# mynameisfiber/baton

Hardware: NVIDIA H100
Metric: federated local samples/sec (whole box), ResNet-18 FedAvg, synthetic non-IID 32x32 shards (higher is better)
Workload: dtype bf16

## Files before the change

### baton_b200/csrc/bindings.cpp

```cpp
#include <ATen/cuda/CUDAContext.h>
#include <c10/cuda/CUDAGuard.h>
#include <torch/extension.h>

#include <optional>
#include <vector>

#include "launch.h"

namespace {

inline cudaStream_t cur_stream() { return at::cuda::getCurrentCUDAStream().stream(); }
inline void check(int rc, const char* what) {
  TORCH_CHECK(rc == 0, "baton_b200::", what, " failed with code ", rc,
              rc > 0 ? std::string(" (") + cudaGetErrorString(static_cast<cudaError_t>(rc)) + ")" : std::string());
}
inline const void* cptr(const at::Tensor& t) { return t.data_ptr(); }
inline void* ptr(at::Tensor& t) { return t.data_ptr(); }
template <class T>
inline T* opt_ptr(const std::optional<at::Tensor>& t) {
  return (t.has_value() && t->defined()) ? reinterpret_cast<T*>(t->data_ptr()) : nullptr;
}
#define CHECK_CUDA(x) TORCH_CHECK((x).is_cuda(), #x " must be a CUDA tensor")

inline const float* prox_anchor(const std::optional<at::Tensor>& anchor, int64_t numel, const at::Tensor& hyper) {
// ... 239 lines not shown
                                static_cast<int>(stride), dgrad ? 1 : 0, static_cast<int>(mc), opt_ptr<float>(col_stats),
                                cur_stream());
  if (rc == -2) return false;
  check(rc, "conv_halo");
  return true;
}
bool conv_igemm_dgrad_s2(const at::Tensor& dy, const at::Tensor& w, at::Tensor dx, int64_t kh, int64_t kw,
                         const std::vector<int64_t>& ntaps, const std::vector<int64_t>& taps, int64_t force_bn) {
  CHECK_CUDA(dy); CHECK_CUDA(w); CHECK_CUDA(dx);
  TORCH_CHECK(dy.scalar_type() == at::kBFloat16 && w.scalar_type() == at::kBFloat16 && dx.scalar_type() == at::kBFloat16 &&
              dy.dim() == 4 && dx.dim() == 4 && dy.is_contiguous() && w.is_contiguous() && dx.is_contiguous());
  TORCH_CHECK(ntaps.size() == 4 && taps.size() == 16, "conv_igemm_dgrad_s2: 4 classes x 4 taps");
  int nt[4], tw[16];
  for (int i = 0; i < 4; ++i) nt[i] = static_cast<int>(ntaps[i]);
  for (int i = 0; i < 16; ++i) tw[i] = static_cast<int>(taps[i]);
  const c10::cuda::CUDAGuard guard(dy.device());
  const int rc = b200_conv_igemm_dgrad_s2(cptr(dy), cptr(w), ptr(dx), static_cast<int>(dx.size(0)),
                                          static_cast<int>(dx.size(1)), static_cast<int>(dx.size(2)),
                                          static_cast<int>(dx.size(3)), static_cast<int>(dy.size(3)), static_cast<int>(kh),
                                          static_cast<int>(kw), static_cast<int>(dy.size(1)), static_cast<int>(dy.size(2)),
                                          nt, tw, static_cast<int>(force_bn), cur_stream());
  if (rc == -2) return false;
  check(rc, "conv_igemm_dgrad_s2");
  return true;
}
bool conv_igemm_wgrad(const at::Tensor& dy, const at::Tensor& x, at::Tensor dw, int64_t cout, int64_t kh, int64_t kw,
                      int64_t stride, int64_t pad, int64_t ho, int64_t wo, int64_t split_k, int64_t force_bn,
                      const std::optional<at::Tensor>& sgd_theta, const std::optional<at::Tensor>& sgd_theta_bf16,
                      const std::optional<at::Tensor>& sgd_mom, const std::optional<at::Tensor>& sgd_hyper,
                      bool sgd_nesterov, const std::optional<at::Tensor>& sgd_anchor,
                      const std::optional<at::Tensor>& sgd_corr, const std::optional<at::Tensor>& sgd_v) {
  CHECK_CUDA(dy); CHECK_CUDA(x); CHECK_CUDA(dw);
  TORCH_CHECK(x.scalar_type() == at::kBFloat16 && dy.scalar_type() == at::kBFloat16 && dw.scalar_type() == at::kFloat &&
              x.dim() == 4 && x.is_contiguous() && dy.is_contiguous());
  const c10::cuda::CUDAGuard guard(x.device());
  const std::optional<B200SgdEpilogue> sgd =
      sgd_epilogue(sgd_theta, sgd_theta_bf16, sgd_mom, sgd_hyper, sgd_nesterov, sgd_anchor, sgd_corr, sgd_v);
  const int rc = b200_conv_igemm_wgrad(cptr(dy), cptr(x), dw.data_ptr<float>(), static_cast<int>(x.size(0)),
                                       static_cast<int>(x.size(1)), static_cast<int>(x.size(2)), static_cast<int>(x.size(3)),
                                       static_cast<int>(cout), static_cast<int>(kh), static_cast<int>(kw),
                                       static_cast<int>(stride), static_cast<int>(pad), static_cast<int>(ho),
                                       static_cast<int>(wo), static_cast<int>(split_k), static_cast<int>(force_bn),
                                       sgd ? &*sgd : nullptr, cur_stream());
  if (rc == -2 || rc == B200_SGD_EPILOGUE_DECLINED) return false;
  check(rc, "conv_igemm_wgrad");
  return true;
// ... 886 lines not shown
  const c10::cuda::CUDAGuard guard(pred.device());
  const int in32 = pred.scalar_type() == at::kFloat;
  const int out32 = dpred.has_value() && dpred->defined() && dpred->scalar_type() == at::kFloat;
  check(b200_mse(pred.data_ptr(), in32, target.data_ptr<float>(), opt_ptr<void>(dpred), out32,
                 loss_acc.data_ptr<float>(), pred.numel(), static_cast<float>(grad_scale), cur_stream()),
        "mse");
}

}

PYBIND11_MODULE(TORCH_EXTENSION_NAME, m) {
  m.doc() = "baton_b200 sm_90a kernels";
  m.attr("MAX_RANKS") = B200_MAX_RANKS;
  m.def("gemm", &gemm);
  m.def("trace_set", &trace_set);
  m.def("attention_fwd", &attention_fwd);
  m.def("attention_bwd", &attention_bwd);
  m.def("bn_bwd_cluster", &bn_bwd_cluster);
  m.def("im2col_tma_probe", &im2col_tma_probe);
  m.def("conv_igemm_fwd", &conv_igemm_fwd);
  m.def("conv_igemm_wgrad", &conv_igemm_wgrad);
  m.def("conv_igemm_dgrad", &conv_igemm_dgrad);
  m.def("conv_igemm_dgrad_s2", &conv_igemm_dgrad_s2);
  m.def("conv_halo", &conv_halo);
  m.def("gemm_batched", &gemm_batched);
  m.def("gemm_fp8", &gemm_fp8);
  m.def("quant_mx_rows", &quant_mx_rows);
  m.def("quant_mx_cols", &quant_mx_cols);
  m.def("fused_sgd", &fused_sgd);
  m.def("fused_sgd_segments", &fused_sgd_segments);
  m.def("weighted_sum", &weighted_sum);
  m.def("fold_client", &fold_client);
  m.def("scaffold_corr", &scaffold_corr);
  m.def("scaffold_dc", &scaffold_dc);
  m.def("cast", &cast);
  m.def("gather_rows", &gather_rows);
  m.def("gather_augment", &gather_augment);
  m.def("gather_mix", &gather_mix);
  m.def("colsum", &colsum);
  m.def("add_bf16", &add_bf16);
  m.def("relu_bwd", &relu_bwd);
  m.def("gelu", &gelu);
  m.def("gelu_bwd", &gelu_bwd);
  m.def("pad_rows", &pad_rows);
  m.def("embedding_bwd", &embedding_bwd);
  m.def("fedavg_allreduce", &fedavg_allreduce);
// ... 41 lines not shown
```

### baton_b200/csrc/gemm_wgmma.cu

```cuda
#define B200_TU_TAG 1
#include "ptx.cuh"
#include "epilogue.cuh"
#include "launch.h"
#include "pdl.cuh"
#include "sgd.cuh"

namespace b200 {

constexpr int BM = 128;
constexpr int BK = 64;
constexpr int WG_K = 16;
constexpr int GEMM_THREADS = 384;
constexpr int CONSUMER_WARPS = 8;
constexpr int CONSUMER_THREADS = 32 * CONSUMER_WARPS;
constexpr int MAX_STAGES = 8;
constexpr int S2_MAX_TAPS = 4;

struct GemmParams {
  int M, N, K;
  void* D;
  long long ldd;
  const float* bias;
  int out_fp32;
  int act;
  float* col_stats;
  int a_mn, b_mn;
  int k_tiles_per_split;
  int atomic_out;
  int cluster_k;
  int stages;
  const uint32_t* tile_flags;
  uint32_t flag_epoch;
  long long flag_elem_off;
  int flag_tile_elems;
  long long flag_bias_off;
  long long ldb;
  float alpha;
  int batched, batch_inner;
  int batch_count;
  long long d_outer, d_inner;
  int conv_ho, conv_wo;
  int conv_stride, conv_pad;
  int conv_kw;
  int conv_cin;
  int conv_taps;
  int conv_ncol;
  const uint32_t* flag_epoch_ptr;
  const float* sgd_hyper = nullptr;
  float* sgd_theta = nullptr;
  __nv_bfloat16* sgd_wb = nullptr;
  float* sgd_mom = nullptr;
  int sgd_nesterov = 0;
  int conv_h = 0, conv_w = 0;
  int s2_ntaps[4] = {0, 0, 0, 0};
  int s2_tap[4][S2_MAX_TAPS] = {};
  const float* bn_scale = nullptr;
  const float* bn_shift = nullptr;
  const __nv_bfloat16* residual = nullptr;
  long long ldr = 0;
  const float* sgd_anchor = nullptr;
  const float* sgd_corr = nullptr;
  float* sgd_v = nullptr;
};

__device__ __forceinline__ void wait_arrival_flags(const uint32_t* flags, long long e0, long long e1, int granule,
                                                   uint32_t need) {
  for (long long t = e0 / granule; t <= e1 / granule; ++t) {
    unsigned long long spins = 0;
    while (static_cast<int32_t>(ld_acquire_sys(flags + t) - need) < 0) {
      if (++spins > (1ull << 26)) break;
    }
  }
}

template <int BN>
struct SmemLayout {
  static constexpr int A_BYTES = BM * BK * 2;
  static constexpr int B_BYTES = BN * BK * 2;
  static constexpr int STAGE_BYTES = A_BYTES + B_BYTES;
  static constexpr int PART_PITCH = BN + 4;
  static constexpr int PART_BYTES = BM * PART_PITCH * 4;
};

__device__ __forceinline__ float apply_act(float v, int act) {
  if (act == 1) return fmaxf(v, 0.f);
// ... 278 lines not shown
  return w;
}
__device__ __forceinline__ int s2_dx_row(const GemmParams& p, int cls, int m) {
  if (m >= p.M) return -1;
  const int hw = p.conv_ho * p.conv_wo;
  const int n = m / hw, r = m - n * hw;
  const int i = r / p.conv_wo, j = r - i * p.conv_wo;
  const int h = 2 * i + (cls >> 1), w = 2 * j + (cls & 1);
  return (h < p.conv_h && w < p.conv_w) ? (n * p.conv_h + h) * p.conv_w + w : -1;
}
template <int BN>
__device__ __forceinline__ void s2_load_ktile(const CUtensorMap* tmA, const CUtensorMap* tmB, const GemmParams& p,
                                              uint8_t* sa, uint8_t* sb, uint64_t* bar, int cls, int kt, int m0, int n0) {
  const int cblocks = p.conv_cin >> 6;
  const int slot = kt / cblocks, cb = kt - slot * cblocks;
  const int tw = s2_tap(p, cls, slot);
  const int q0 = m0 % p.conv_wo, t0 = m0 / p.conv_wo;
  tma_load_im2col_4d(sa, tmA, bar, cb * 64, q0, t0 % p.conv_ho, t0 / p.conv_ho, (tw >> 24) & 0xff, (tw >> 16) & 0xff);
  const int wcol = (tw & 0xffff) * p.conv_ncol + n0;
#pragma unroll
  for (int j = 0; j < BN / 64; ++j) tma_load_2d(sb + j * 8192, tmB, bar, wcol + j * 64, cb * 64);
}

template <int BN, int STAGES, int CONV = 0, bool SGD = false, bool AFFINE = false, bool PROX = false, bool SCAF = false,
          bool ADAM = false>
__global__ void __launch_bounds__(GEMM_THREADS, 1)
gemm_bf16_fixed_kernel(const __grid_constant__ CUtensorMap tmA, const __grid_constant__ CUtensorMap tmB,
                         const GemmParams p) {
  using L = SmemLayout<BN>;
  static_assert(STAGES * L::STAGE_BYTES >= L::PART_BYTES, "the drained ring must hold the fp32 accumulator tile");
  extern __shared__ __align__(1024) uint8_t smem_raw[];
  uint8_t* smem = reinterpret_cast<uint8_t*>((reinterpret_cast<uintptr_t>(smem_raw) + 1023) & ~uintptr_t(1023));
  uint64_t* full_bar = reinterpret_cast<uint64_t*>(smem + STAGES * L::STAGE_BYTES);
  uint64_t* empty_bar = full_bar + STAGES;
  float* cstat = reinterpret_cast<float*>(empty_bar + STAGES);

  griddep_launch_dependents();
  const int warp = threadIdx.x >> 5;
  int m0 = blockIdx.y * BM;
  const int cls = CONV == 4 ? s2_class(p, m0) : 0;
  const int n0 = blockIdx.x * BN;
  const int k_tiles_total = CONV == 4 ? s2_ntaps(p, cls) * (p.conv_cin >> 6) : (p.K + BK - 1) / BK;
  const int bz_outer = p.batched ? static_cast<int>(blockIdx.z) / p.batch_inner : 0;
  const int bz_inner = p.batched ? static_cast<int>(blockIdx.z) % p.batch_inner : 0;
  const int kt_begin = p.batched ? 0 : blockIdx.z * p.k_tiles_per_split;
  int kt_end = kt_begin + p.k_tiles_per_split;
  if (kt_end > k_tiles_total) kt_end = k_tiles_total;
  const int num_kt = kt_end - kt_begin;

  if (warp == 0 && elect_one()) {
    tma_prefetch_desc(&tmA);
    tma_prefetch_desc(&tmB);
    for (int s = 0; s < STAGES; ++s) {
      mbar_init(&full_bar[s], 1);
      mbar_init(&empty_bar[s], CONSUMER_WARPS);
    }
    fence_barrier_init();
  }
  __syncthreads();
  griddep_wait();

  if (warp == 0) {
    if (elect_one()) {
      if (p.tile_flags != nullptr) {
        const int rows_here = (p.N - n0) < BN ? (p.N - n0) : BN;
// ... 17 lines not shown
        if constexpr (CONV == 2) {
          const int live = (p.N - n0 + 63) / 64 < BN / 64 ? (p.N - n0 + 63) / 64 : BN / 64;
          mbar_expect_tx(&full_bar[s], L::A_BYTES + live * 8192);
        } else {
          mbar_expect_tx(&full_bar[s], L::STAGE_BYTES);
        }
        if (p.batched) {
          if (!p.a_mn) {
            tma_load_4d(sa, &tmA, &full_bar[s], k0, m0, bz_inner, bz_outer);
          } else {
#pragma unroll
            for (int j = 0; j < BM / 64; ++j)
              tma_load_4d(sa + j * 8192, &tmA, &full_bar[s], m0 + j * 64, k0, bz_inner, bz_outer);
          }
          if (!p.b_mn) {
            tma_load_4d(sb, &tmB, &full_bar[s], k0, n0, bz_inner, bz_outer);
          } else {
#pragma unroll
            for (int j = 0; j < BN / 64; ++j)
              tma_load_4d(sb + j * 8192, &tmB, &full_bar[s], n0 + j * 64, k0, bz_inner, bz_outer);
          }
        } else if constexpr (CONV == 4) {
          s2_load_ktile<BN>(&tmA, &tmB, p, sa, sb, &full_bar[s], cls, kt_begin + i, m0, n0);
        } else {
        if constexpr (CONV == 1 || CONV == 3) {
          const int kt = kt_begin + i;
          const int cblocks = p.conv_cin >> 6;
          const int tap = kt / cblocks, cb = kt - tap * cblocks;
          const int fr = tap / p.conv_kw, fs = tap - fr * p.conv_kw;
          const int q0 = m0 % p.conv_wo, t0 = m0 / p.conv_wo;
          tma_load_im2col_4d(sa, &tmA, &full_bar[s], cb * 64, q0 * p.conv_stride - p.conv_pad,
                             (t0 % p.conv_ho) * p.conv_stride - p.conv_pad, t0 / p.conv_ho, fs, fr);
        } else if (!p.a_mn) {
          tma_load_2d(sa, &tmA, &full_bar[s], k0, m0);
        } else {
#pragma unroll
          for (int j = 0; j < BM / 64; ++j)
            tma_load_2d(sa + j * 8192, &tmA, &full_bar[s], m0 + j * 64, k0);
        }
        if constexpr (CONV == 2) {
          const int q0 = k0 % p.conv_wo, t0 = k0 / p.conv_wo;
          const int w0 = q0 * p.conv_stride - p.conv_pad, h0 = (t0 % p.conv_ho) * p.conv_stride - p.conv_pad;
          const int img = t0 / p.conv_ho;
#pragma unroll
          for (int j = 0; j < BN / 64; ++j) {
            const int col = n0 + j * 64;
// ... 15 lines not shown
        } else {
#pragma unroll
          for (int j = 0; j < BN / 64; ++j) tma_load_2d(sb + j * 8192, &tmB, &full_bar[s], n0 + j * 64, k0);
        }
        }
      }
    }
  } else if (warp >= 4) {
    const int ew = warp - 4;
    float acc[BN / 2];
    int s = 0;
    uint32_t ph = 0;
    consume_ktiles<BN>(acc, smem, STAGES, full_bar, empty_bar, s, ph, num_kt, p.a_mn, p.b_mn, ew >> 2);
    if (threadIdx.x == 128) TRACE_POINT();
    named_bar_sync(1, CONSUMER_THREADS);
    float* part = reinterpret_cast<float*>(smem);
    wg_store_acc<BN>(acc, part, L::PART_PITCH, 64 * (ew >> 2));
    named_bar_sync(1, CONSUMER_THREADS);
    const int q = ew & 3;
    constexpr int NCHUNK = BN / 32;
    const int c_begin = (ew < 4 ? 0 : (NCHUNK + 1) / 2) * 32, c_end = (ew < 4 ? (NCHUNK + 1) / 2 : NCHUNK) * 32;
    const int lrow = q * 32 + static_cast<int>(lane_id());
    const int row = m0 + lrow;
    const int orow = CONV == 4 ? s2_dx_row(p, cls, row) : row;
    const bool row_ok = CONV == 4 ? orow >= 0 : row < p.M;
    const size_t elt = p.out_fp32 ? 4 : 2;
    uint8_t* drow = reinterpret_cast<uint8_t*>(p.D) +
                    (static_cast<size_t>(CONV == 4 && orow < 0 ? 0 : orow) * p.ldd + static_cast<size_t>(bz_outer) * p.d_outer +
                     static_cast<size_t>(bz_inner) * p.d_inner) * elt;
    const bool vec_ok = ((reinterpret_cast<uintptr_t>(p.D) & 15) == 0) && ((p.ldd * elt) % 16 == 0);
    const bool sgd_vec = SGD && (p.ldd % 4 == 0) &&
                         ((reinterpret_cast<uintptr_t>(p.sgd_theta) | reinterpret_cast<uintptr_t>(p.sgd_mom) |
                           (PROX ? reinterpret_cast<uintptr_t>(p.sgd_anchor) : 0) |
                           (SCAF ? reinterpret_cast<uintptr_t>(p.sgd_corr) : 0) |
                           (ADAM ? reinterpret_cast<uintptr_t>(p.sgd_v) : 0)) & 15) == 0 &&
                         (reinterpret_cast<uintptr_t>(p.sgd_wb) & 7) == 0;
    float* sstat = cstat + q * 2 * BN;
    const bool want_stats = p.col_stats != nullptr;
#pragma unroll 1
    for (int c = c_begin; c < c_end; c += 32) {
      uint32_t r[32];
      acc_ld_row32(part + lrow * L::PART_PITCH + c, r);
      const int col0 = n0 + c;
      float v[32];
#pragma unroll
      for (int j = 0; j < 32; ++j) v[j] = __uint_as_float(r[j]);
      if (col0 >= p.N) {
        if (want_stats) { sstat[c + lane_id()] = 0.f; sstat[BN + c + lane_id()] = 0.f; }
        continue;
      }
      if constexpr (AFFINE) {
// ... 230 lines not shown
      epilogue_tile<BN>(p, acc_tile, ew & 3, ew >> 2, m0, n0, epi_stage + ew * EPI_WARP_BYTES,
                        vec_ok && ((d_off * elt) & 15) == 0, d_off);
    }
  }
}


template <int BN, bool CLUSTER, int CONV = 0, bool AFFINE = false>
__global__ void __launch_bounds__(GEMM_THREADS, 1)
gemm_bf16_splitk_kernel(const __grid_constant__ CUtensorMap tmA, const __grid_constant__ CUtensorMap tmB,
                        const GemmParams p) {
  using L = SmemLayout<BN>;
  extern __shared__ __align__(1024) uint8_t smem_raw[];
  uint8_t* smem = reinterpret_cast<uint8_t*>((reinterpret_cast<uintptr_t>(smem_raw) + 1023) & ~uintptr_t(1023));
  const int STAGES = p.stages;
  const int ring_bytes = STAGES * L::STAGE_BYTES;
  const int data_bytes = L::PART_BYTES > ring_bytes ? L::PART_BYTES : ring_bytes;
  uint64_t* full_bar = reinterpret_cast<uint64_t*>(smem + data_bytes);
  uint64_t* empty_bar = full_bar + MAX_STAGES;
  float* cstat = reinterpret_cast<float*>(empty_bar + MAX_STAGES);

  griddep_launch_dependents();
  const int warp = threadIdx.x >> 5;
  const int m0 = blockIdx.y * BM;
  const int n0 = blockIdx.x * BN;
  const int k_tiles_total = (p.K + BK - 1) / BK;
  const int kt_begin = blockIdx.z * p.k_tiles_per_split;
  int kt_end = kt_begin + p.k_tiles_per_split;
  if (kt_end > k_tiles_total) kt_end = k_tiles_total;
  const int num_kt = kt_end - kt_begin;

  if (warp == 0 && elect_one()) {
    tma_prefetch_desc(&tmA);
    tma_prefetch_desc(&tmB);
    for (int s = 0; s < STAGES; ++s) {
      mbar_init(&full_bar[s], 1);
      mbar_init(&empty_bar[s], CONSUMER_WARPS);
    }
    fence_barrier_init();
  }
  __syncthreads();
  griddep_wait();

  if (warp == 0) {
    if (elect_one()) {
      if (p.tile_flags != nullptr) {
        const int rows_here = (p.N - n0) < BN ? (p.N - n0) : BN;
        const uint32_t need = p.flag_epoch_ptr != nullptr ? *reinterpret_cast<const volatile uint32_t*>(p.flag_epoch_ptr)
                                                          : p.flag_epoch;
        wait_arrival_flags(p.tile_flags, p.flag_elem_off + static_cast<long long>(n0) * p.ldb,
                           p.flag_elem_off + static_cast<long long>(n0 + rows_here) * p.ldb - 1, p.flag_tile_elems, need);
        if (p.flag_bias_off >= 0)
          wait_arrival_flags(p.tile_flags, p.flag_bias_off + n0, p.flag_bias_off + n0 + rows_here - 1,
                             p.flag_tile_elems, need);
        fence_proxy_async_all();
      }
      int s = 0;
      uint32_t ph = 0;
      for (int i = 0; i < num_kt; ++i) {
        mbar_wait(&empty_bar[s], ph ^ 1);
        uint8_t* sa = smem + s * L::STAGE_BYTES;
        uint8_t* sb = sa + L::A_BYTES;
        const int k0 = (kt_begin + i) * BK;
        mbar_expect_tx(&full_bar[s], L::STAGE_BYTES);
        if constexpr (CONV == 1 || CONV == 3) {
          const int kt = kt_begin + i;
          const int cblocks = p.conv_cin >> 6;
          const int tap = kt / cblocks, cb = kt - tap * cblocks;
          const int fr = tap / p.conv_kw, fs = tap - fr * p.conv_kw;
          const int q0 = m0 % p.conv_wo, t0 = m0 / p.conv_wo;
          tma_load_im2col_4d(sa, &tmA, &full_bar[s], cb * 64, q0 * p.conv_stride - p.conv_pad,
                             (t0 % p.conv_ho) * p.conv_stride - p.conv_pad, t0 / p.conv_ho, fs, fr);
        } else if (!p.a_mn) {
          tma_load_2d(sa, &tmA, &full_bar[s], k0, m0);
        } else {
#pragma unroll
          for (int j = 0; j < BM / 64; ++j)
            tma_load_2d(sa + j * 8192, &tmA, &full_bar[s], m0 + j * 64, k0);
        }
        if constexpr (CONV == 3) {
          const int kt = kt_begin + i;
          const int cblocks = p.conv_cin >> 6;
          const int tap = kt / cblocks, cb = kt - tap * cblocks;
          const int wcol = (p.conv_taps - 1 - tap) * p.conv_ncol + n0;
#pragma unroll
          for (int j = 0; j < BN / 64; ++j) tma_load_2d(sb + j * 8192, &tmB, &full_bar[s], wcol + j * 64, cb * 64);
        } else if (!p.b_mn) {
          tma_load_2d(sb, &tmB, &full_bar[s], k0, n0);
        } else {
#pragma unroll
          for (int j = 0; j < BN / 64; ++j) tma_load_2d(sb + j * 8192, &tmB, &full_bar[s], n0 + j * 64, k0);
        }
        if (++s == STAGES) { s = 0; ph ^= 1; }
      }
    }
  } else if (warp >= 4) {
    const int ew = warp - 4;
    float acc[BN / 2];
    int s = 0;
    uint32_t ph = 0;
    consume_ktiles<BN>(acc, smem, STAGES, full_bar, empty_bar, s, ph, num_kt, p.a_mn, p.b_mn, ew >> 2);
    named_bar_sync(1, CONSUMER_THREADS);
    float* part = reinterpret_cast<float*>(smem);
    wg_store_acc<BN>(acc, part, L::PART_PITCH, 64 * (ew >> 2));
    if constexpr (!CLUSTER) {
      named_bar_sync(1, CONSUMER_THREADS);
      const int q = ew & 3;
      constexpr int NCHUNK = BN / 32;
      const int c_begin = (ew < 4 ? 0 : (NCHUNK + 1) / 2) * 32, c_end = (ew < 4 ? (NCHUNK + 1) / 2 : NCHUNK) * 32;
      const int lrow = q * 32 + static_cast<int>(lane_id());
      const int row = m0 + lrow;
      const size_t elt = p.out_fp32 ? 4 : 2;
      const bool vec_ok = ((reinterpret_cast<uintptr_t>(p.D) & 15) == 0) && ((p.ldd * elt) % 16 == 0);
#pragma unroll 1
      for (int c = c_begin; c < c_end; c += 32) {
        const int col0 = n0 + c;
        if (row >= p.M || col0 >= p.N) continue;
        uint32_t r[32];
        acc_ld_row32(part + lrow * L::PART_PITCH + c, r);
        float v[32];
#pragma unroll
        for (int j = 0; j < 32; ++j) v[j] = __uint_as_float(r[j]);
        store_row_chunk<32, AFFINE>(p, row, col0, v, vec_ok);
      }
    }
  }

  if constexpr (CLUSTER) {
    const int S = p.cluster_k;
    cluster_sync_all();
    if (warp >= 4 && warp < 8) {
      const uint32_t me = cluster_ctarank();
      const int rows_per = BM / S;
      constexpr int CG = BN / 8;
      const int t = threadIdx.x - 128;
      const size_t elt = p.out_fp32 ? 4 : 2;
      const bool vec_ok = ((reinterpret_cast<uintptr_t>(p.D) & 15) == 0) && ((p.ldd * elt) % 16 == 0);
      const bool want_stats = p.col_stats != nullptr;
      float cs[8] = {0.f, 0.f, 0.f, 0.f, 0.f, 0.f, 0.f, 0.f}, cq[8] = {0.f, 0.f, 0.f, 0.f, 0.f, 0.f, 0.f, 0.f};
      for (int item = t; item < rows_per * CG; item += 128) {
        const int lrow = static_cast<int>(me) * rows_per + item / CG;
        const int c = (item % CG) * 8;
        const uint32_t laddr = smem_u32(smem) + static_cast<uint32_t>((lrow * L::PART_PITCH + c) * 4);
        float v[8] = {0.f, 0.f, 0.f, 0.f, 0.f, 0.f, 0.f, 0.f};
        for (int r = 0; r < S; ++r) {
          const float4 a = ld_dsmem_f4(laddr, r), b = ld_dsmem_f4(laddr + 16, r);
          v[0] += a.x; v[1] += a.y; v[2] += a.z; v[3] += a.w;
          v[4] += b.x; v[5] += b.y; v[6] += b.z; v[7] += b.w;
        }
        const int row = m0 + lrow, col0 = n0 + c;
        if (want_stats) {
#pragma unroll
          for (int j = 0; j < 8; ++j) {
            const float rnd = __bfloat162float(__float2bfloat16_rn(v[j]));
            cs[j] += rnd;
            cq[j] = fmaf(rnd, rnd, cq[j]);
          }
        }
        if (row < p.M && col0 < p.N) store_row_chunk<8, AFFINE>(p, row, col0, v, vec_ok);
      }
      if (want_stats) {
#pragma unroll
        for (int j = 0; j < 8; ++j) {
#pragma unroll
          for (int o = CG; o < 32; o <<= 1) {
            cs[j] += __shfl_xor_sync(0xffffffffu, cs[j], o);
            cq[j] += __shfl_xor_sync(0xffffffffu, cq[j], o);
          }
        }
        const int wq = t >> 5, ln = t & 31;
        if (ln < CG) {
#pragma unroll
          for (int j = 0; j < 8; ++j) {
            cstat[wq * 2 * BN + ln * 8 + j] = cs[j];
            cstat[wq * 2 * BN + BN + ln * 8 + j] = cq[j];
          }
        }
        named_bar_sync(2, 128);
        for (int i = t; i < 2 * BN; i += 128) {
          const int col = i < BN ? i : i - BN;
          if (n0 + col < p.N) {
            const float v = cstat[i] + cstat[2 * BN + i] + cstat[4 * BN + i] + cstat[6 * BN + i];
            atomicAdd(p.col_stats + (i < BN ? 0 : p.N) + n0 + col, v);
          }
        }
      }
    }
    cluster_sync_all();
  }
}


typedef CUresult (*EncodeTiledFn)(CUtensorMap*, CUtensorMapDataType, cuuint32_t, void*, const cuuint64_t*,
                                  const cuuint64_t*, const cuuint32_t*, const cuuint32_t*, CUtensorMapInterleave,
                                  CUtensorMapSwizzle, CUtensorMapL2promotion, CUtensorMapFloatOOBfill);

static EncodeTiledFn get_encode_fn() {
  static thread_local bool ctx_bound = false;
  if (!ctx_bound) {
    cudaFree(nullptr);
    ctx_bound = true;
  }
  static EncodeTiledFn fn = nullptr;
  if (fn == nullptr) {
    void* ptr = nullptr;
    cudaDriverEntryPointQueryResult qres;
    cudaError_t e = cudaGetDriverEntryPoint("cuTensorMapEncodeTiled", &ptr, cudaEnableDefault, &qres);
    if (e != cudaSuccess || qres != cudaDriverEntryPointSuccess || ptr == nullptr) return nullptr;
    fn = reinterpret_cast<EncodeTiledFn>(ptr);
  }
// ... 439 lines not shown
  }
  if (max_taps == 0) return -2;
  const int bn = clamp_bn(force_bn > 0 ? force_bn : (Cin > 64 ? 128 : 64));
  CUtensorMap ta, tb;
  int rc = b200_encode_map_im2col_bf16(&ta, dy, N, Ho, Wo, Cout, 1, 1, 1, 0, 64, BM);
  if (rc) return rc;
  rc = make_map(&tb, w, Cout, static_cast<long long>(KH) * KW * Cin, static_cast<long long>(KH) * KW * Cin, 64, BK);
  if (rc) return rc;
  const int k_tiles = max_taps * (Cout / 64);
  p.M = static_cast<int>(M); p.N = Cin; p.K = k_tiles * BK; p.D = dx; p.ldd = Cin; p.bias = nullptr; p.out_fp32 = 0;
  p.act = 0; p.a_mn = 0; p.b_mn = 1; p.k_tiles_per_split = k_tiles; p.cluster_k = 1; p.atomic_out = 0;
  p.col_stats = nullptr;
  p.tile_flags = nullptr; p.flag_epoch = 0; p.alpha = 1.0f; p.flag_elem_off = 0; p.flag_tile_elems = 0;
  p.ldb = static_cast<long long>(KH) * KW * Cin;
  p.flag_bias_off = -1; p.flag_epoch_ptr = nullptr;
  p.batched = 0; p.batch_inner = 1; p.batch_count = 1; p.d_outer = 0; p.d_inner = 0;
  p.conv_ho = Ho; p.conv_wo = Wo; p.conv_stride = 2; p.conv_pad = 0; p.conv_kw = KW; p.conv_cin = Cout;
  p.conv_taps = KH * KW; p.conv_ncol = Cin; p.conv_h = H; p.conv_w = W;
  dim3 grid((Cin + bn - 1) / bn, static_cast<unsigned>(4 * tiles_m), 1);
  if (bn == 128) return launch_fixed<128, 6, 4>(ta, tb, p, grid, stream);
  return launch_fixed<64, 8, 4>(ta, tb, p, grid, stream);
}

extern "C" int b200_conv_igemm_wgrad(const void* dy, const void* x, float* dw, int N, int H, int W, int Cin, int Cout,
                                     int KH, int KW, int stride, int pad, int Ho, int Wo, int split_k, int force_bn,
                                     const B200SgdEpilogue* sgd, cudaStream_t stream) {
  using namespace b200;
  const long long Mp = static_cast<long long>(N) * Ho * Wo;
  const int Kc = KH * KW * Cin;
  if (Mp <= 0 || Cout <= 0) return 0;
  if (Cin % 64 != 0 || Cout % 8 != 0 || Mp > (1ll << 30) || (reinterpret_cast<uintptr_t>(x) & 15) ||
      (reinterpret_cast<uintptr_t>(dy) & 15) || (reinterpret_cast<uintptr_t>(dw) & 15))
    return -2;
  const int bn = clamp_bn(force_bn > 0 ? force_bn : (Kc > 64 ? 128 : 64));
  CUtensorMap ta, tb;
  int rc = make_map(&ta, dy, Mp, Cout, Cout, 64, BK);
  if (rc) return rc;
  rc = b200_encode_map_im2col_bf16(&tb, x, N, H, W, Cin, KH, KW, stride, pad, 64, 64);
  if (rc) return rc;
  const int k_tiles = static_cast<int>((Mp + BK - 1) / BK);
  if (split_k < 1) split_k = 1;
  if (split_k > k_tiles) split_k = k_tiles;
  const int per = (k_tiles + split_k - 1) / split_k;
  split_k = (k_tiles + per - 1) / per;
  if (sgd != nullptr && split_k != 1) return B200_SGD_EPILOGUE_DECLINED;
  GemmParams p;
// ... 21 lines not shown
```

### baton_b200/csrc/launch.h

```cpp
#pragma once
#include <cuda_runtime.h>
#include <stdint.h>

#define B200_MAX_RANKS 16

extern "C" {

struct B200SgdEpilogue {
  float* theta;
  void* theta_bf16;
  float* mom;
  const float* hyper;
  int nesterov;
  const float* anchor;
  const float* corr;
  float* v;
};
#define B200_SGD_EPILOGUE_DECLINED (-6)

struct B200AffineEpilogue {
  const float* scale;
  const float* shift;
  const void* residual;
  long long ldr;
// ... 1 lines not shown
};
#define B200_AFFINE_EPILOGUE_DECLINED (-7)

int b200_gemm_bf16(const void* a, const void* b, void* d, const float* bias, int M, int N, int K, long long lda,
                   long long ldb, long long ldd, int a_mn, int b_mn, int out_fp32, int act, int split_k, int accumulate,
                   float alpha, const uint32_t* tile_flags, uint32_t flag_epoch, long long flag_elem_off, int flag_tile_elems,
                   long long flag_bias_off, int force_bn, float* col_stats, const uint32_t* flag_epoch_ptr,
                   const B200SgdEpilogue* sgd, const B200AffineEpilogue* affine, cudaStream_t stream);
int b200_gemm_bf16_batched(const void* a, const void* b, void* d, int M, int N, int K, long long lda, long long ldb,
                           long long ldd, int a_mn, int b_mn, int out_fp32, int act, float alpha, int n_outer,
                           int n_inner, long long a_outer, long long a_inner, long long b_outer, long long b_inner,
                           long long d_outer, long long d_inner, int accumulate, cudaStream_t stream);
int b200_attention_fwd(const void* qkv, void* out, void* probs, int B, int S, int H, int dh, float scale,
                       cudaStream_t stream);
int b200_attention_bwd(const void* qkv, const void* dout, const void* probs, void* dqkv, int B, int S, int H, int dh,
                       float scale, cudaStream_t stream);
int b200_conv_igemm_fwd(const void* x, const void* w, void* y, int N, int H, int W, int Cin, int Cout, int KH, int KW,
                        int stride, int pad, int Ho, int Wo, int cluster_k, int force_bn, float* col_stats,
                        const B200AffineEpilogue* affine, cudaStream_t stream);
int b200_conv_igemm_dgrad(const void* dy, const void* w, void* dx, int N, int H, int W, int Cin, int Cout, int KH, int KW,
                          int pad, int Ho, int Wo, int cluster_k, int force_bn, cudaStream_t stream);
int b200_conv_igemm_dgrad_s2(const void* dy, const void* w, void* dx, int N, int H, int W, int Cin, int Cout, int KH,
                             int KW, int Ho, int Wo, const int* ntaps, const int* taps, int force_bn, cudaStream_t stream);
int b200_conv_igemm_wgrad(const void* dy, const void* x, float* dw, int N, int H, int W, int Cin, int Cout, int KH, int KW,
                          int stride, int pad, int Ho, int Wo, int split_k, int force_bn, const B200SgdEpilogue* sgd,
                          cudaStream_t stream);
int b200_conv_halo(const void* src, const void* w, void* out, int N, int H, int W, int C, int Nout, int stride,
                   int dgrad, int mc, float* col_stats, cudaStream_t stream);
int b200_im2col_tma_probe(const void* x, void* col, int N, int H, int W, int C, int KH, int KW, int stride, int pad,
                          int Ho, int Wo, cudaStream_t stream);
int b200_gemm_fp8(const void* a, const void* b, void* d, const float* bias, const void* sfa, const void* sfb, int M, int N,
                  int K, long long lda, long long ldb, long long ldd, int out_fp32, int act, int split_k, int accumulate,
                  float alpha, cudaStream_t stream);
int b200_quant_mx_rows(const void* x, void* q, void* sf, long long R, int C, long long ld_in, int Cp, cudaStream_t stream);
int b200_quant_mx_cols(const void* x, void* q, void* sf, long long R, int C, long long ld_in, long long Rp,
                       cudaStream_t stream);
int b200_gemm_simt(const void* a, const void* b, void* d, const float* bias, int M, int N, int K, long long lda,
                   long long ldb, long long ldd, int a_mn, int b_mn, int out_fp32, int act, int accumulate,
                   float alpha, cudaStream_t stream);

int b200_fused_sgd(float* w, float* g, float* mom, void* w_bf16, long long n, const float* hyper, int zero_grad,
                   int nesterov, const unsigned long long* wire_slot, const float* pack_global,
                   const float* pack_scale, long long n_pack, int wire_fp32, const float* prox_anchor,
                   const float* corr, float* adam_v, cudaStream_t stream);
int b200_fused_sgd_segments(float* w, float* g, float* mom, void* w_bf16, const long long* segments, int n_seg,
                            const float* hyper, int nesterov, const float* prox_anchor, const float* corr,
// ... 192 lines not shown
```

### baton_b200/ops/functional.py

```python
from __future__ import annotations

import collections
import functools
from typing import List, Optional, Sequence, Tuple

import torch

from ._ext import load

BF16 = torch.bfloat16
NUM_SMS = 132


def _pitch(t: torch.Tensor) -> int:
    assert t.dim() == 2 and (t.stride(1) == 1 or t.shape[1] == 1), "GEMM operand must have unit inner stride"
    return t.stride(0) if t.shape[0] > 1 else max(t.stride(0), t.shape[1])


def _tma_ok(t: torch.Tensor) -> bool:
    return t.dtype == BF16 and _pitch(t) % 8 == 0 and t.data_ptr() % 16 == 0


def pick_bn(M: int, N: int) -> int:
    m_tiles = (M + 127) // 128
# ... 387 lines not shown


def halo_smem_bytes(h: int, w: int, c: int = 64, stride: int = 1) -> int:
    ho, wo = conv_out_size(h, 3, stride, 1), conv_out_size(w, 3, stride, 1)
    box = (HALO_BM // (ho * wo)) * (stride * (ho - 1) + 3) * (stride * (wo - 1) + 3) * 128
    k_tiles = 9 * (c // 64)
    return c // 64 * round_up(box, 1024) + k_tiles * 8192 + round_up(1 + k_tiles, 16) * 8 + 4 * 64 * 4 + 1024


def halo_eligible(kh: int, kw: int, stride: int, pad: int, c: int, h: int, w: int,
                  affine: Optional[dict] = None, dgrad: bool = False) -> bool:
    if kh != 3 or kw != 3 or pad != 1 or (stride, c) not in _HALO_FORMS or (dgrad and stride != 1):
        return False
    hw = conv_out_size(h, 3, stride, 1) * conv_out_size(w, 3, stride, 1)
    return (hw <= HALO_BM and HALO_BM % hw == 0 and affine is None and
            halo_smem_bytes(h, w, c, stride) <= _HALO_MAX_SMEM)


def halo_cluster(m_rows: int) -> int:
    tiles = (m_rows + HALO_BM - 1) // HALO_BM
    return 4 if tiles % 4 == 0 else 2 if tiles % 2 == 0 else 1


def _conv_path(path: Optional[str], eligible: bool) -> str:
    if path is None:
        return "halo" if eligible else "im2col"
    if path not in ("halo", "im2col"):
        raise ValueError("path must be None, 'halo' or 'im2col', not {!r}".format(path))
    if path == "halo" and not eligible:
        raise ValueError("the halo kernel does not take this convolution (see halo_eligible)")
    return path


def conv_igemm_fwd(x: torch.Tensor, w2d: torch.Tensor, kh: int, kw: int, stride: int, pad: int,
                   col_stats: Optional[torch.Tensor] = None, affine: Optional[dict] = None,
                   cluster_k: Optional[int] = None, force_bn: int = 0,
                   out: Optional[torch.Tensor] = None, path: Optional[str] = None,
                   mc: Optional[int] = None) -> Optional[torch.Tensor]:
    n, h, w, c = x.shape
    cout = w2d.shape[0]
    if c % 64 or w2d.shape[1] != kh * kw * c or not x.is_contiguous() or not w2d.is_contiguous():
        return None
    ho, wo = conv_out_size(h, kh, stride, pad), conv_out_size(w, kw, stride, pad)
    M, K = n * ho * wo, kh * kw * c
    halo = halo_eligible(kh, kw, stride, pad, c, h, w, affine) and cout % 8 == 0
    if _conv_path(path, halo) == "halo":
        y = out if out is not None else torch.empty((M, cout), dtype=BF16, device=x.device)
        if not load().conv_halo(x, w2d, y, stride, False, mc or halo_cluster(M), col_stats):
            raise RuntimeError("conv_halo declined a convolution halo_eligible admits")
        return y
    bn = force_bn or pick_bn(M, cout)
    if cluster_k is None:
        cluster_k = pick_cluster_k(M, cout, K, bn)
    y = out if out is not None else torch.empty((M, cout), dtype=BF16, device=x.device)
    af = affine or {}
    ok = load().conv_igemm_fwd(x, w2d, y, kh, kw, stride, pad, ho, wo, cluster_k, bn, col_stats, af.get("scale"),
                               af.get("shift"), af.get("residual"), bool(af.get("relu", False)))
    return y if ok else None


S2_MAX_TAPS = 4


def conv_s2_dgrad_taps(kh: int, kw: int, pad: int, ho: int, wo: int) -> Optional[List[List[Tuple[int, int, int]]]]:
    classes = []
    for a in (0, 1):
        for b in (0, 1):
            taps = []
            for r in range(kh):
                if (a + pad - r) % 2:
                    continue
                dp = (a + pad - r) // 2
                for s in range(kw):
                    if (b + pad - s) % 2:
                        continue
                    dq = (b + pad - s) // 2
                    if dp < 0 or dq < 0:
                        return None
                    if dp < ho and dq < wo:
                        taps.append((r * kw + s, dp, dq))
            if len(taps) > S2_MAX_TAPS:
                return None
            classes.append(taps)
    return classes


def conv_igemm_dgrad(dy: torch.Tensor, w2d: torch.Tensor, in_shape, kh: int, kw: int, pad: int, stride: int = 1,
                     out: Optional[torch.Tensor] = None, path: Optional[str] = None,
                     mc: Optional[int] = None, cluster_k: Optional[int] = None) -> Optional[torch.Tensor]:
    n, h, w, c = in_shape
    cout = dy.shape[-1]
    if c % 64 or cout % 64 or w2d.shape[1] != kh * kw * c or not dy.is_contiguous() or not w2d.is_contiguous():
        return None
    if _conv_path(path, halo_eligible(kh, kw, stride, pad, cout, h, w, dgrad=True)) == "halo":
        dx = out if out is not None else torch.empty((n, h, w, c), dtype=BF16, device=dy.device)
        if not load().conv_halo(dy, w2d, dx, 1, True, mc or halo_cluster(n * h * w), None):
            raise RuntimeError("conv_halo declined a convolution halo_eligible admits")
        return dx
    if stride == 1:
        M, K = n * h * w, kh * kw * cout
        bn = pick_bn(M, c)
        dx = out if out is not None else torch.empty((n, h, w, c), dtype=BF16, device=dy.device)
        if cluster_k is None:
            cluster_k = pick_cluster_k(M, c, K, bn)
        ok = load().conv_igemm_dgrad(dy, w2d, dx, kh, kw, pad, cluster_k, bn)
        return dx if ok else None
    if stride != 2:
        return None
    ho, wo = dy.shape[1], dy.shape[2]
    classes = conv_s2_dgrad_taps(kh, kw, pad, ho, wo)
    if classes is None:
        return None
    bn = pick_bn(4 * n * ho * wo, c)
    words = [[t | dp << 16 | dq << 24 for t, dp, dq in taps] + [0] * (S2_MAX_TAPS - len(taps)) for taps in classes]
    dx = out if out is not None else torch.empty((n, h, w, c), dtype=BF16, device=dy.device)
    ok = load().conv_igemm_dgrad_s2(dy, w2d, dx, kh, kw, [len(t) for t in classes], [x for ws in words for x in ws], bn)
    return dx if ok else None


def conv_igemm_wgrad_(dy2d: torch.Tensor, x: torch.Tensor, dw2d: torch.Tensor, kh: int, kw: int, stride: int,
# ... 184 lines not shown
```

Before: 225,700.

## Add tap-table conv kernel for tiny spatial 3x3 convs skipping padded taps

Adds a new CONV==5 mode in the wgmma implicit-GEMM kernel that, for 3x3 pad-1 convolutions with output at most 2x2, precomputes per-output-pixel lists of valid (tap, pixel) pairs. Each output pixel class loads only the K tiles for taps that land inside the image, so the zero-padding taps an im2col GEMM would multiply are never touched. Forward and stride-1 dgrad are routed to it by default when the halo path does not apply, using cluster split-K of 4. In exchange it adds a per-tile table lookup and extra grid rows per class, and it covers only the small late ResNet layers.

```diff
diff --git a/baton_b200/csrc/bindings.cpp b/baton_b200/csrc/bindings.cpp
--- a/baton_b200/csrc/bindings.cpp
+++ b/baton_b200/csrc/bindings.cpp
@@ -285,6 +285,34 @@
                                           nt, tw, static_cast<int>(force_bn), cur_stream());
   if (rc == -2) return false;
   check(rc, "conv_igemm_dgrad_s2");
+  return true;
+}
+bool conv_taps(const at::Tensor& src, const at::Tensor& w, at::Tensor out, int64_t ho, int64_t wo, bool dgrad,
+               const std::vector<int64_t>& ntaps, const std::vector<int64_t>& taps, int64_t cluster_k, int64_t force_bn,
+               const std::optional<at::Tensor>& col_stats) {
+  CHECK_CUDA(src); CHECK_CUDA(w); CHECK_CUDA(out);
+  TORCH_CHECK(src.scalar_type() == at::kBFloat16 && w.scalar_type() == at::kBFloat16 && out.scalar_type() == at::kBFloat16 &&
+              src.dim() == 4 && src.is_contiguous() && w.is_contiguous() && out.is_contiguous());
+  TORCH_CHECK(ho >= 1 && wo >= 1 && ho * wo <= 4 && ntaps.size() == static_cast<size_t>(ho * wo) && taps.size() == 16,
+              "conv_taps: one tap count per output pixel (at most 2x2) and 4 x 4 tap words");
+  const int64_t rows = src.size(0) * ho * wo;
+  TORCH_CHECK(rows > 0 && out.numel() % rows == 0, "conv_taps: out must hold [N*Ho*Wo, Nout] elements");
+  const int64_t nout = out.numel() / rows;
+  TORCH_CHECK(w.numel() == 9 * src.size(3) * nout, "conv_taps: w must be [Cout, 9*Cin]");
+  TORCH_CHECK(dgrad ? !col_stats.has_value()
+                    : (!col_stats.has_value() || (col_stats->scalar_type() == at::kFloat && col_stats->numel() >= 2 * nout)),
+              "conv_taps: col_stats is a [2 Cout] fp32 buffer of the forward");
+  int nt[4] = {0, 0, 0, 0}, tw[16];
+  for (size_t i = 0; i < ntaps.size(); ++i) nt[i] = static_cast<int>(ntaps[i]);
+  for (int i = 0; i < 16; ++i) tw[i] = static_cast<int>(taps[i]);
+  const c10::cuda::CUDAGuard guard(src.device());
+  const int rc = b200_conv_taps(cptr(src), cptr(w), ptr(out), static_cast<int>(src.size(0)), static_cast<int>(src.size(1)),
+                                static_cast<int>(src.size(2)), static_cast<int>(src.size(3)), static_cast<int>(nout),
+                                static_cast<int>(ho), static_cast<int>(wo), dgrad ? 1 : 0, nt, tw,
+                                static_cast<int>(cluster_k), static_cast<int>(force_bn), opt_ptr<float>(col_stats),
+                                cur_stream());
+  if (rc == -2) return false;
+  check(rc, "conv_taps");
   return true;
 }
 bool conv_igemm_wgrad(const at::Tensor& dy, const at::Tensor& x, at::Tensor dw, int64_t cout, int64_t kh, int64_t kw,
@@ -1217,6 +1245,7 @@
   m.def("conv_igemm_wgrad", &conv_igemm_wgrad);
   m.def("conv_igemm_dgrad", &conv_igemm_dgrad);
   m.def("conv_igemm_dgrad_s2", &conv_igemm_dgrad_s2);
+  m.def("conv_taps", &conv_taps);
   m.def("conv_halo", &conv_halo);
   m.def("gemm_batched", &gemm_batched);
   m.def("gemm_fp8", &gemm_fp8);
diff --git a/baton_b200/csrc/gemm_wgmma.cu b/baton_b200/csrc/gemm_wgmma.cu
--- a/baton_b200/csrc/gemm_wgmma.cu
+++ b/baton_b200/csrc/gemm_wgmma.cu
@@ -15,6 +15,8 @@
 constexpr int CONSUMER_THREADS = 32 * CONSUMER_WARPS;
 constexpr int MAX_STAGES = 8;
 constexpr int S2_MAX_TAPS = 4;
+constexpr int TAPS_MAX_CLASSES = 4;
+constexpr int TAPS_MAX = 4;
 
 struct GemmParams {
   int M, N, K;
@@ -61,6 +63,8 @@
   const float* sgd_anchor = nullptr;
   const float* sgd_corr = nullptr;
   float* sgd_v = nullptr;
+  int taps_n[TAPS_MAX_CLASSES] = {};
+  int taps_tab[TAPS_MAX_CLASSES][TAPS_MAX] = {};
 };
 
 __device__ __forceinline__ void wait_arrival_flags(const uint32_t* flags, long long e0, long long e1, int granule,
@@ -385,6 +389,40 @@
   for (int j = 0; j < BN / 64; ++j) tma_load_2d(sb + j * 8192, tmB, bar, wcol + j * 64, cb * 64);
 }
 
+__device__ __forceinline__ int taps_count(const GemmParams& p, int cls) {
+  int n = 0;
+#pragma unroll
+  for (int c = 0; c < TAPS_MAX_CLASSES; ++c) n = c == cls ? p.taps_n[c] : n;
+  return n;
+}
+__device__ __forceinline__ int taps_entry(const GemmParams& p, int cls, int slot) {
+  int w = 0;
+#pragma unroll
+  for (int c = 0; c < TAPS_MAX_CLASSES; ++c)
+#pragma unroll
+    for (int t = 0; t < TAPS_MAX; ++t) w = (c == cls && t == slot) ? p.taps_tab[c][t] : w;
+  return w;
+}
+__device__ __forceinline__ int taps_out_row(const GemmParams& p, int cls, int m) {
+  return m < p.M ? m * (p.conv_ho * p.conv_wo) + cls : -1;
+}
+template <int BN>
+__device__ __forceinline__ void taps_load_ktile(const CUtensorMap* tmA, const CUtensorMap* tmB, const GemmParams& p,
+                                                uint8_t* sa, uint8_t* sb, uint64_t* bar, int cls, int kt, int m0, int n0) {
+  const int cblocks = p.conv_cin >> 6;
+  const int slot = kt / cblocks, cb = kt - slot * cblocks;
+  const int e = taps_entry(p, cls, slot);
+  const int tap = e & 0xff, pix = e >> 8;
+  tma_load_2d(sa, tmA, bar, pix * p.conv_cin + cb * 64, m0);
+  if (!p.b_mn) {
+    tma_load_2d(sb, tmB, bar, tap * p.conv_cin + cb * 64, n0);
+  } else {
+    const int wcol = tap * p.conv_ncol + n0;
+#pragma unroll
+    for (int j = 0; j < BN / 64; ++j) tma_load_2d(sb + j * 8192, tmB, bar, wcol + j * 64, cb * 64);
+  }
+}
+
 template <int BN, int STAGES, int CONV = 0, bool SGD = false, bool AFFINE = false, bool PROX = false, bool SCAF = false,
           bool ADAM = false>
 __global__ void __launch_bounds__(GEMM_THREADS, 1)
@@ -401,9 +439,11 @@
   griddep_launch_dependents();
   const int warp = threadIdx.x >> 5;
   int m0 = blockIdx.y * BM;
-  const int cls = CONV == 4 ? s2_class(p, m0) : 0;
+  const int cls = CONV == 4 || CONV == 5 ? s2_class(p, m0) : 0;
   const int n0 = blockIdx.x * BN;
-  const int k_tiles_total = CONV == 4 ? s2_ntaps(p, cls) * (p.conv_cin >> 6) : (p.K + BK - 1) / BK;
+  const int k_tiles_total = CONV == 4   ? s2_ntaps(p, cls) * (p.conv_cin >> 6)
+                            : CONV == 5 ? taps_count(p, cls) * (p.conv_cin >> 6)
+                                        : (p.K + BK - 1) / BK;
   const int bz_outer = p.batched ? static_cast<int>(blockIdx.z) / p.batch_inner : 0;
   const int bz_inner = p.batched ? static_cast<int>(blockIdx.z) % p.batch_inner : 0;
   const int kt_begin = p.batched ? 0 : blockIdx.z * p.k_tiles_per_split;
@@ -467,6 +507,8 @@
           }
         } else if constexpr (CONV == 4) {
           s2_load_ktile<BN>(&tmA, &tmB, p, sa, sb, &full_bar[s], cls, kt_begin + i, m0, n0);
+        } else if constexpr (CONV == 5) {
+          taps_load_ktile<BN>(&tmA, &tmB, p, sa, sb, &full_bar[s], cls, kt_begin + i, m0, n0);
         } else {
         if constexpr (CONV == 1 || CONV == 3) {
           const int kt = kt_begin + i;
@@ -528,11 +570,11 @@
     const int c_begin = (ew < 4 ? 0 : (NCHUNK + 1) / 2) * 32, c_end = (ew < 4 ? (NCHUNK + 1) / 2 : NCHUNK) * 32;
     const int lrow = q * 32 + static_cast<int>(lane_id());
     const int row = m0 + lrow;
-    const int orow = CONV == 4 ? s2_dx_row(p, cls, row) : row;
-    const bool row_ok = CONV == 4 ? orow >= 0 : row < p.M;
+    const int orow = CONV == 4 ? s2_dx_row(p, cls, row) : CONV == 5 ? taps_out_row(p, cls, row) : row;
+    const bool row_ok = CONV == 4 || CONV == 5 ? orow >= 0 : row < p.M;
     const size_t elt = p.out_fp32 ? 4 : 2;
     uint8_t* drow = reinterpret_cast<uint8_t*>(p.D) +
-                    (static_cast<size_t>(CONV == 4 && orow < 0 ? 0 : orow) * p.ldd + static_cast<size_t>(bz_outer) * p.d_outer +
+                    (static_cast<size_t>((CONV == 4 || CONV == 5) && orow < 0 ? 0 : orow) * p.ldd + static_cast<size_t>(bz_outer) * p.d_outer +
                      static_cast<size_t>(bz_inner) * p.d_inner) * elt;
     const bool vec_ok = ((reinterpret_cast<uintptr_t>(p.D) & 15) == 0) && ((p.ldd * elt) % 16 == 0);
     const bool sgd_vec = SGD && (p.ldd % 4 == 0) &&
@@ -809,13 +851,14 @@
 
   griddep_launch_dependents();
   const int warp = threadIdx.x >> 5;
-  const int m0 = blockIdx.y * BM;
+  int m0 = blockIdx.y * BM;
+  const int cls = CONV == 5 ? s2_class(p, m0) : 0;
   const int n0 = blockIdx.x * BN;
-  const int k_tiles_total = (p.K + BK - 1) / BK;
+  const int k_tiles_total = CONV == 5 ? taps_count(p, cls) * (p.conv_cin >> 6) : (p.K + BK - 1) / BK;
   const int kt_begin = blockIdx.z * p.k_tiles_per_split;
   int kt_end = kt_begin + p.k_tiles_per_split;
   if (kt_end > k_tiles_total) kt_end = k_tiles_total;
-  const int num_kt = kt_end - kt_begin;
+  const int num_kt = CONV == 5 && kt_end < kt_begin ? 0 : kt_end - kt_begin;
 
   if (warp == 0 && elect_one()) {
     tma_prefetch_desc(&tmA);
@@ -843,6 +886,7 @@
         fence_proxy_async_all();
       }
       int s = 0;
+      TRACE_POINT();
       uint32_t ph = 0;
       for (int i = 0; i < num_kt; ++i) {
         mbar_wait(&empty_bar[s], ph ^ 1);
@@ -850,6 +894,9 @@
         uint8_t* sb = sa + L::A_BYTES;
         const int k0 = (kt_begin + i) * BK;
         mbar_expect_tx(&full_bar[s], L::STAGE_BYTES);
+        if constexpr (CONV == 5) {
+          taps_load_ktile<BN>(&tmA, &tmB, p, sa, sb, &full_bar[s], cls, kt_begin + i, m0, n0);
+        } else {
         if constexpr (CONV == 1 || CONV == 3) {
           const int kt = kt_begin + i;
           const int cblocks = p.conv_cin >> 6;
@@ -878,6 +925,7 @@
 #pragma unroll
           for (int j = 0; j < BN / 64; ++j) tma_load_2d(sb + j * 8192, &tmB, &full_bar[s], n0 + j * 64, k0);
         }
+        }
         if (++s == STAGES) { s = 0; ph ^= 1; }
       }
     }
@@ -887,6 +935,7 @@
     int s = 0;
     uint32_t ph = 0;
     consume_ktiles<BN>(acc, smem, STAGES, full_bar, empty_bar, s, ph, num_kt, p.a_mn, p.b_mn, ew >> 2);
+    if (threadIdx.x == 128) TRACE_POINT();
     named_bar_sync(1, CONSUMER_THREADS);
     float* part = reinterpret_cast<float*>(smem);
     wg_store_acc<BN>(acc, part, L::PART_PITCH, 64 * (ew >> 2));
@@ -908,7 +957,7 @@
         float v[32];
 #pragma unroll
         for (int j = 0; j < 32; ++j) v[j] = __uint_as_float(r[j]);
-        store_row_chunk<32, AFFINE>(p, row, col0, v, vec_ok);
+        store_row_chunk<32, AFFINE>(p, CONV == 5 ? taps_out_row(p, cls, row) : row, col0, v, vec_ok);
       }
     }
   }
@@ -916,6 +965,7 @@
   if constexpr (CLUSTER) {
     const int S = p.cluster_k;
     cluster_sync_all();
+    if (threadIdx.x == 128) TRACE_POINT();
     if (warp >= 4 && warp < 8) {
       const uint32_t me = cluster_ctarank();
       const int rows_per = BM / S;
@@ -944,7 +994,8 @@
             cq[j] = fmaf(rnd, rnd, cq[j]);
           }
         }
-        if (row < p.M && col0 < p.N) store_row_chunk<8, AFFINE>(p, row, col0, v, vec_ok);
+        if (row < p.M && col0 < p.N)
+          store_row_chunk<8, AFFINE>(p, CONV == 5 ? taps_out_row(p, cls, row) : row, col0, v, vec_ok);
       }
       if (want_stats) {
 #pragma unroll
@@ -973,6 +1024,7 @@
         }
       }
     }
+    if (threadIdx.x == 128) TRACE_POINT();
     cluster_sync_all();
   }
 }
@@ -1458,6 +1510,56 @@
   return launch_fixed<64, 8, 4>(ta, tb, p, grid, stream);
 }
 
+extern "C" int b200_conv_taps(const void* src, const void* w, void* out, int N, int H, int W, int C, int Nout, int Ho,
+                              int Wo, int dgrad, const int* ntaps, const int* taps, int cluster_k, int force_bn,
+                              float* col_stats, cudaStream_t stream) {
+  using namespace b200;
+  const int classes = Ho * Wo;
+  if (N <= 0) return 0;
+  if (C % 64 != 0 || Nout % 64 != 0 || Ho < 1 || Wo < 1 || classes > TAPS_MAX_CLASSES || (dgrad && col_stats != nullptr) ||
+      (dgrad && (Ho != H || Wo != W)) || (reinterpret_cast<uintptr_t>(src) & 15) || (reinterpret_cast<uintptr_t>(w) & 15) ||
+      (reinterpret_cast<uintptr_t>(out) & 15))
+    return -2;
+  if (cluster_k != 1 && cluster_k != 2 && cluster_k != 4 && cluster_k != 8) return -5;
+  const long long tiles_m = (static_cast<long long>(N) + BM - 1) / BM;
+  if (classes * tiles_m > 65535) return -2;
+  GemmParams p;
+  int max_taps = 0;
+  for (int c = 0; c < classes; ++c) {
+    if (ntaps[c] < 1 || ntaps[c] > TAPS_MAX) return -2;
+    for (int t = 0; t < ntaps[c]; ++t) {
+      const int e = taps[c * TAPS_MAX + t];
+      if (e < 0 || (e & 0xff) >= 9 || (e >> 8) >= H * W) return -2;
+      p.taps_tab[c][t] = e;
+    }
+    p.taps_n[c] = ntaps[c];
+    max_taps = ntaps[c] > max_taps ? ntaps[c] : max_taps;
+  }
+  const int bn = clamp_bn(force_bn > 0 ? force_bn : 64);
+  const int cin = dgrad ? Nout : C;
+  CUtensorMap ta, tb;
+  int rc = make_map(&ta, src, N, static_cast<long long>(H) * W * C, static_cast<long long>(H) * W * C, BK, BM);
+  if (rc) return rc;
+  rc = dgrad ? make_map(&tb, w, C, 9ll * cin, 9ll * cin, 64, BK) : make_map(&tb, w, Nout, 9ll * cin, 9ll * cin, BK, bn);
+  if (rc) return rc;
+  const int k_tiles = max_taps * (C / 64);
+  while (cluster_k > 1 && (cluster_k - 1) * ((k_tiles + cluster_k - 1) / cluster_k) >= k_tiles) cluster_k >>= 1;
+  const int per = (k_tiles + cluster_k - 1) / cluster_k;
+  p.M = N; p.N = Nout; p.K = k_tiles * BK; p.D = out; p.ldd = Nout; p.bias = nullptr; p.out_fp32 = 0; p.act = 0;
+  p.a_mn = 0; p.b_mn = dgrad ? 1 : 0; p.k_tiles_per_split = per; p.cluster_k = cluster_k; p.atomic_out = 0;
+  p.col_stats = col_stats;
+  p.tile_flags = nullptr; p.flag_epoch = 0; p.alpha = 1.0f; p.flag_elem_off = 0; p.flag_tile_elems = 0; p.ldb = 9ll * cin;
+  p.flag_bias_off = -1; p.flag_epoch_ptr = nullptr;
+  p.batched = 0; p.batch_inner = 1; p.batch_count = 1; p.d_outer = 0; p.d_inner = 0;
+  const int max_stages = bn == 128 ? 6 : 8;
+  p.stages = per < max_stages ? (per < 2 ? 2 : per) : max_stages;
+  p.conv_ho = Ho; p.conv_wo = Wo; p.conv_stride = 1; p.conv_pad = 0; p.conv_kw = 3; p.conv_cin = C;
+  p.conv_taps = 9; p.conv_ncol = cin;
+  dim3 grid((Nout + bn - 1) / bn, static_cast<unsigned>(classes * tiles_m), cluster_k);
+  if (cluster_k > 1) return bn == 128 ? launch_cfg<128, 5>(ta, tb, p, grid, stream) : launch_cfg<64, 5>(ta, tb, p, grid, stream);
+  return bn == 128 ? launch_fixed<128, 6, 5>(ta, tb, p, grid, stream) : launch_fixed<64, 8, 5>(ta, tb, p, grid, stream);
+}
+
 extern "C" int b200_conv_igemm_wgrad(const void* dy, const void* x, float* dw, int N, int H, int W, int Cin, int Cout,
                                      int KH, int KW, int stride, int pad, int Ho, int Wo, int split_k, int force_bn,
                                      const B200SgdEpilogue* sgd, cudaStream_t stream) {
diff --git a/baton_b200/csrc/launch.h b/baton_b200/csrc/launch.h
--- a/baton_b200/csrc/launch.h
+++ b/baton_b200/csrc/launch.h
@@ -47,6 +47,9 @@
                           int pad, int Ho, int Wo, int cluster_k, int force_bn, cudaStream_t stream);
 int b200_conv_igemm_dgrad_s2(const void* dy, const void* w, void* dx, int N, int H, int W, int Cin, int Cout, int KH,
                              int KW, int Ho, int Wo, const int* ntaps, const int* taps, int force_bn, cudaStream_t stream);
+int b200_conv_taps(const void* src, const void* w, void* out, int N, int H, int W, int C, int Nout, int Ho, int Wo,
+                   int dgrad, const int* ntaps, const int* taps, int cluster_k, int force_bn, float* col_stats,
+                   cudaStream_t stream);
 int b200_conv_igemm_wgrad(const void* dy, const void* x, float* dw, int N, int H, int W, int Cin, int Cout, int KH, int KW,
                           int stride, int pad, int Ho, int Wo, int split_k, int force_bn, const B200SgdEpilogue* sgd,
                           cudaStream_t stream);
diff --git a/baton_b200/ops/functional.py b/baton_b200/ops/functional.py
--- a/baton_b200/ops/functional.py
+++ b/baton_b200/ops/functional.py
@@ -433,14 +433,73 @@
     return 4 if tiles % 4 == 0 else 2 if tiles % 2 == 0 else 1
 
 
-def _conv_path(path: Optional[str], eligible: bool) -> str:
+TAPS_MAX = 4
+TAPS_CLASSES = 4
+
+
+def conv_taps_table(kh: int, kw: int, stride: int, pad: int, h: int, w: int,
+                     dgrad: bool = False) -> List[List[Tuple[int, int]]]:
+    ho, wo = (h, w) if dgrad else (conv_out_size(h, kh, stride, pad), conv_out_size(w, kw, stride, pad))
+    off = kh - 1 - pad if dgrad else pad
+    classes = []
+    for i in range(ho):
+        for j in range(wo):
+            taps = []
+            for t in range(kh * kw):
+                r, s = divmod(t, kw)
+                hs, ws = i * (1 if dgrad else stride) - off + r, j * (1 if dgrad else stride) - off + s
+                if 0 <= hs < h and 0 <= ws < w:
+                    taps.append((kh * kw - 1 - t if dgrad else t, hs * w + ws))
+            classes.append(taps)
+    return classes
+
+
+@functools.lru_cache(maxsize=None)
+def _taps_words(stride: int, h: int, w: int, dgrad: bool) -> Tuple[List[int], List[int]]:
+    table = conv_taps_table(3, 3, stride, 1, h, w, dgrad)
+    if len(table) > TAPS_CLASSES or max(len(t) for t in table) > TAPS_MAX:
+        raise ValueError("not a tap-table convolution (see taps_eligible)")
+    words = [0] * (TAPS_CLASSES * TAPS_MAX)
+    for c, taps in enumerate(table):
+        for t, (tap, pix) in enumerate(taps):
+            words[c * TAPS_MAX + t] = tap | pix << 8
+    return [len(t) for t in table], words
+
+
+def taps_eligible(kh: int, kw: int, stride: int, pad: int, c: int, h: int, w: int, cout: int,
+                  affine: Optional[dict] = None, dgrad: bool = False) -> bool:
+    if kh != 3 or kw != 3 or pad != 1 or stride not in (1, 2) or (dgrad and stride != 1):
+        return False
+    if c % 64 or cout % 64 or affine is not None or (h == 1 and w == 1):
+        return False
+    ho, wo = conv_out_size(h, 3, stride, 1), conv_out_size(w, 3, stride, 1)
+    if ho > 2 or wo > 2 or (stride == 2 and ho * wo > 1):
+        return False
+    return not halo_eligible(kh, kw, stride, pad, cout if dgrad else c, h, w, dgrad=dgrad)
+
+
+TAPS_CLUSTER_K = 4
+
+
+def _conv_path(path: Optional[str], eligible: bool, taps: bool = False) -> str:
     if path is None:
-        return "halo" if eligible else "im2col"
-    if path not in ("halo", "im2col"):
-        raise ValueError("path must be None, 'halo' or 'im2col', not {!r}".format(path))
+        return "halo" if eligible else "taps" if taps else "im2col"
+    if path not in ("halo", "taps", "im2col"):
+        raise ValueError("path must be None, 'halo', 'taps' or 'im2col', not {!r}".format(path))
     if path == "halo" and not eligible:
         raise ValueError("the halo kernel does not take this convolution (see halo_eligible)")
+    if path == "taps" and not taps:
+        raise ValueError("the tap-table kernel does not take this convolution (see taps_eligible)")
     return path
+
+
+def _conv_taps(src: torch.Tensor, w2d: torch.Tensor, out: torch.Tensor, stride: int, ho: int, wo: int, dgrad: bool,
+               cluster_k: Optional[int], force_bn: int, col_stats: Optional[torch.Tensor]) -> None:
+    _, h, w, _ = src.shape
+    ntaps, words = _taps_words(stride, h, w, dgrad)
+    ck = cluster_k or TAPS_CLUSTER_K
+    if not load().conv_taps(src, w2d, out, ho, wo, dgrad, ntaps, words, ck, force_bn, col_stats):
+        raise RuntimeError("conv_taps declined a convolution taps_eligible admits")
 
 
 def conv_igemm_fwd(x: torch.Tensor, w2d: torch.Tensor, kh: int, kw: int, stride: int, pad: int,
@@ -455,10 +514,15 @@
     ho, wo = conv_out_size(h, kh, stride, pad), conv_out_size(w, kw, stride, pad)
     M, K = n * ho * wo, kh * kw * c
     halo = halo_eligible(kh, kw, stride, pad, c, h, w, affine) and cout % 8 == 0
-    if _conv_path(path, halo) == "halo":
+    route = _conv_path(path, halo, taps_eligible(kh, kw, stride, pad, c, h, w, cout, affine))
+    if route == "halo":
         y = out if out is not None else torch.empty((M, cout), dtype=BF16, device=x.device)
         if not load().conv_halo(x, w2d, y, stride, False, mc or halo_cluster(M), col_stats):
             raise RuntimeError("conv_halo declined a convolution halo_eligible admits")
+        return y
+    if route == "taps":
+        y = out if out is not None else torch.empty((M, cout), dtype=BF16, device=x.device)
+        _conv_taps(x, w2d, y, stride, ho, wo, False, cluster_k, force_bn, col_stats)
         return y
     bn = force_bn or pick_bn(M, cout)
     if cluster_k is None:
@@ -498,15 +562,22 @@
 
 def conv_igemm_dgrad(dy: torch.Tensor, w2d: torch.Tensor, in_shape, kh: int, kw: int, pad: int, stride: int = 1,
                      out: Optional[torch.Tensor] = None, path: Optional[str] = None,
-                     mc: Optional[int] = None, cluster_k: Optional[int] = None) -> Optional[torch.Tensor]:
+                     mc: Optional[int] = None, cluster_k: Optional[int] = None,
+                     force_bn: int = 0) -> Optional[torch.Tensor]:
     n, h, w, c = in_shape
     cout = dy.shape[-1]
     if c % 64 or cout % 64 or w2d.shape[1] != kh * kw * c or not dy.is_contiguous() or not w2d.is_contiguous():
         return None
-    if _conv_path(path, halo_eligible(kh, kw, stride, pad, cout, h, w, dgrad=True)) == "halo":
+    route = _conv_path(path, halo_eligible(kh, kw, stride, pad, cout, h, w, dgrad=True),
+                       taps_eligible(kh, kw, stride, pad, c, h, w, cout, dgrad=True))
+    if route == "halo":
         dx = out if out is not None else torch.empty((n, h, w, c), dtype=BF16, device=dy.device)
         if not load().conv_halo(dy, w2d, dx, 1, True, mc or halo_cluster(n * h * w), None):
             raise RuntimeError("conv_halo declined a convolution halo_eligible admits")
+        return dx
+    if route == "taps":
+        dx = out if out is not None else torch.empty((n, h, w, c), dtype=BF16, device=dy.device)
+        _conv_taps(dy, w2d, dx, 1, h, w, True, cluster_k, force_bn, None)
         return dx
     if stride == 1:
         M, K = n * h * w, kh * kw * cout
```

Result: faster. 230,200 (median of 6 runs) (+2.0%).
